# showlab/VideoSwap

Measured on AMD Instinct MI355X. Metric: denoised frames/sec, 16-frame 512x512 clip @ 50 DDIM steps (end to end: inversion + CFG sampling), higher is better.
Workload: dtype f16; 1 GPU; BASELINE.json configs[1]: 16-frame 512x512 clip, SD-1.5 UNet3D + AnimateDiff motion modules, 50-step DDIM inversion (B=1) + 50-step CFG-7.5 DDIM sampling (B=2), 1 clip per GPU per step; launch=eager, parallelism=clip-parallel x1

## Files before the change

videoswap_amd/csrc/gemm.hip:

```cpp
#include "gemm_common.h"
#include "prof.h"
#include <algorithm>
#include <cstdlib>
#include <stdlib.h>
#include <string.h>

using namespace vsxg;

static long tile_tune() { return vsxg::gemm_option("tile_tune"); }
static long force_tile() { return tile_tune() & 15; }
static bool tune_deep() { return (tile_tune() & 16) != 0; }
static int tune_splits() { return (int)((tile_tune() >> 8) & 15); }

namespace {


#ifdef VSX_GEMM_TIMING
#define TSTAMP(i) do { const long t_now = (long)clock64(); t_seg[i] += t_now - t_last; t_last = t_now; } while (0)
#else
#define TSTAMP(i) do { } while (0)
#endif

template <int BM, int BN, int WAVES_M, int WAVES_N, bool SWAP, int NSTAGE>
__global__ __launch_bounds__(WAVES_M* WAVES_N * 64) void gemm_kernel(const GemmParams p) {
    constexpr int PREFETCH = NSTAGE - 1;
    constexpr int NW = WAVES_M * WAVES_N;
    constexpr int WM = BM / WAVES_M, WN = BN / WAVES_N;
    constexpr int TM = WM / 32, TN = WN / 32;
    constexpr int A_BLKS = BM / 8, B_BLKS = BN / 8;
    static_assert(A_BLKS % NW == 0, "A blocks must split evenly over the waves");
    constexpr int GA = A_BLKS / NW;
    constexpr int GB_LO = B_BLKS / NW, GB_HI = (B_BLKS + NW - 1) / NW;
    constexpr int N_HI = B_BLKS - GB_LO * NW;
    constexpr int STAGE = (BM + BN) * 128;

    extern __shared__ __attribute__((aligned(16))) unsigned char smem[];

    const int tid = threadIdx.x;
    const int lane = tid & 63;
    const int wave = __builtin_amdgcn_readfirstlane(tid >> 6);
    const int wr = wave / WAVES_N, wc = wave % WAVES_N;
    const int l31 = lane & 31, hi = lane >> 5;
#ifdef VSX_GEMM_TIMING
    const long t_begin = (long)clock64();
#endif

    int tile_n, tile_m, split;
    if (p.xcd_gm > 0) {
        const int xcd = blockIdx.x & 7, local = blockIdx.x >> 3;
        const int gm = p.xcd_gm;
        const int RB = p.tiles_m / gm;
        const int CB = (p.tiles_n * (p.splitk > 1 ? p.splitk : 1)) / (8 / gm);
        const int lr = local % RB;
        const int np = (xcd / gm) * CB + local / RB;
        tile_m = (xcd % gm) * RB + lr;
        tile_n = np % p.tiles_n;
        split = np / p.tiles_n;
    } else {
        int wg = blockIdx.x;
        const int nwg = gridDim.x, q = nwg >> 3, r = nwg & 7;
        const int xcd = wg & 7, local = wg >> 3;
        wg = (xcd < r ? xcd * (q + 1) : r * (q + 1) + (xcd - r) * q) + local;
        tile_n = wg % p.tiles_n;
        tile_m = wg / p.tiles_n;
        split = p.splitk > 1 ? (int)blockIdx.z : 0;
    }
    const long m0 = (long)tile_m * BM;
    const long n0 = p.geglu ? (long)tile_n * (BN / 2) : (long)tile_n * BN;

    const int z = (p.splitk > 1 || p.xcd_gm > 0) ? 0 : (int)blockIdx.z;
    const int z0 = z / p.batch1, z1 = z - z0 * p.batch1;
    const half_t* Ab = p.A + z0 * p.a_bs0 + z1 * p.a_bs1;
    const half_t* Bb = p.B + z0 * p.b_bs0 + z1 * p.b_bs1;

    constexpr int OOB_OFF = (int)0x80000000;
    const int lrow = lane >> 3;
    const int pslot = lane & 7;
    const int kofs_e = (pslot ^ (lrow >> 1)) * 8;
    const int kofs_o = (pslot ^ (4 | (lrow >> 1))) * 8;

    const __amdgpu_buffer_rsrc_t rsrcA =
        __builtin_amdgcn_make_buffer_rsrc(const_cast<half_t*>(Ab), 0, (int)p.a_bytes, 0x00020000);
    const __amdgpu_buffer_rsrc_t rsrcA2 =
        __builtin_amdgcn_make_buffer_rsrc(const_cast<half_t*>(p.A2 ? p.A2 : p.A), 0, (int)p.a2_bytes, 0x00020000);
    const __amdgpu_buffer_rsrc_t rsrcB =
        __builtin_amdgcn_make_buffer_rsrc(const_cast<half_t*>(Bb), 0, (int)p.b_bytes, 0x00020000);

    bool a_ok[GA];
    int a_h0[GA], a_w0[GA], a_ibase[GA], a_kofs[GA];
    int va[GA];
    const int Hs = p.ups ? (p.H >> 1) : p.H;
    const int Ws = p.ups ? (p.W >> 1) : p.W;
    const int pad = p.pad;
#pragma unroll
    for (int i = 0; i < GA; ++i) {
        const long m = m0 + (wave * GA + i) * 8 + lrow;
        a_ok[i] = m < p.M;
        a_h0[i] = 0; a_w0[i] = 0; a_ibase[i] = 0;
        a_kofs[i] = ((wave * GA + i) & 1) ? kofs_o : kofs_e;
        va[i] = a_ok[i] ? (int)((m * p.lda + a_kofs[i]) * 2) : OOB_OFF;
        if (p.a_mode == 1) {
            const long hw = (long)p.Ho * p.Wo;
            const long mm = a_ok[i] ? m : 0;
            const int img = (int)(mm / hw);
            const int rem = (int)(mm - (long)img * hw);
            const int ho = rem / p.Wo;
            a_h0[i] = ho * p.stride - pad;
            a_w0[i] = (rem - ho * p.Wo) * p.stride - pad;
            a_ibase[i] = img * Hs;
        }
    }
    const int gbw = wave < N_HI ? GB_HI : GB_LO;
    const int b_blk0 = wave < N_HI ? wave * GB_HI : N_HI * GB_HI + (wave - N_HI) * GB_LO;
    int vb[GB_HI], b_kofs[GB_HI];
#pragma unroll
    for (int j = 0; j < GB_HI; ++j) {
        const int jr = (b_blk0 + j) * 8 + lrow;
        b_kofs[j] = ((b_blk0 + j) & 1) ? kofs_o : kofs_e;
        long n;
        bool ok;
        if (p.geglu) {
            const long oc = n0 + (jr >> 5) * 16 + (jr & 15);
            ok = oc < p.N;
            n = oc + ((jr & 16) ? p.N : 0);
        } else {
            n = n0 + jr;
            ok = n < p.N;
        }
        vb[j] = (ok && j < gbw) ? (int)((n * p.ldb + b_kofs[j]) * 2) : OOB_OFF;
    }

    const int Ctot = p.C1 + p.C2;
    const int nk = (int)((p.K + BK - 1) / BK);
    const int ktail_from = (int)(p.K - (long)(nk - 1) * BK);
    const bool fast_tap = p.a_mode == 1 && (Ctot % BK == 0) && (p.C1 % BK == 0);
    const int kt_begin = split * p.nk_per;
    const int kt_end = p.splitk > 1 ? min(nk, kt_begin + p.nk_per) : nk;
    int t_kh = 0, t_kw = 0, t_c = 0;
    bool t_second = false, t_dirty = true;
    if (fast_tap && kt_begin > 0) {
        const int k0 = kt_begin * BK;
        const int tap = k0 / Ctot, rem = k0 - tap * Ctot;
        t_kh = tap / p.ks;
        t_kw = tap - t_kh * p.ks;
        t_second = rem >= p.C1;
        t_c = t_second ? rem - p.C1 : rem;
    }

    unsigned char* i_sb = smem;
    bool i_tail = false, i_second = false;
    int i_soffA = 0, i_soffB = 0;
    auto issue_prep = [&](int kt, int stage) {
        unsigned char* sb = smem + stage * STAGE;
        const bool last_tail = (kt == nk - 1) && ktail_from < BK;
        int soffA = kt * (BK * 2), soffB = kt * (BK * 2);
        bool second = false;
        if (p.a_mode == 1) {
            if (fast_tap) {
                if (t_dirty) {
                    const int cs = t_second ? p.C2 : p.C1;
#pragma unroll
                    for (int i = 0; i < GA; ++i) {
                        const int hh = a_h0[i] + t_kh, ww = a_w0[i] + t_kw;
                        const bool ok = a_ok[i] && (unsigned)hh < (unsigned)p.H && (unsigned)ww < (unsigned)p.W;
                        const int hsrc = p.ups ? (hh >> 1) : hh, wsrc = p.ups ? (ww >> 1) : ww;
                        va[i] = ok ? (((a_ibase[i] + hsrc) * Ws + wsrc) * cs + a_kofs[i]) * 2 : OOB_OFF;
                    }
                    t_dirty = false;
                }
                second = t_second;
                soffA = t_c * 2;
                t_c += BK;
                if (t_c >= (t_second ? p.C2 : p.C1)) {
                    t_c = 0;
                    t_dirty = true;
                    if (!t_second && p.C2 > 0) {
                        t_second = true;
                    } else {
                        t_second = false;
                        if (++t_kw == p.ks) { t_kw = 0; ++t_kh; }
                    }
                }
            } else {
#pragma unroll
                for (int i = 0; i < GA; ++i) {
                    const long k = (long)kt * BK + a_kofs[i];
                    const int kk = k < p.K ? (int)k : 0;
                    const int tap = kk / Ctot;
                    const int ci = kk - tap * Ctot;
                    const int kh = tap / p.ks, kw = tap - kh * p.ks;
                    const int hh = a_h0[i] + kh, ww = a_w0[i] + kw;
                    const bool ok = a_ok[i] && k < p.K && (unsigned)hh < (unsigned)p.H && (unsigned)ww < (unsigned)p.W;
                    const int hsrc = p.ups ? (hh >> 1) : hh, wsrc = p.ups ? (ww >> 1) : ww;
                    va[i] = ok ? (((a_ibase[i] + hsrc) * Ws + wsrc) * p.C1 + ci) * 2 : OOB_OFF;
                }
                soffA = 0;
            }
        }
        i_sb = sb; i_tail = last_tail; i_second = second; i_soffA = soffA; i_soffB = soffB;
    };
    constexpr int NPIECE = GA + GB_HI;
    bool i_on = true;
    bool i_gate = true;
    auto issue_piece = [&](const int q) {
        if (!(i_on && i_gate)) return;
        if (q < GA) {
            const int qi = q < GA ? q : 0;
            const int v = (i_tail && a_kofs[qi] >= ktail_from) ? OOB_OFF : va[qi];
            lptr_t dst = (lptr_t)(i_sb + (wave * GA + q) * 1024);
            if (i_second)
                __builtin_amdgcn_raw_ptr_buffer_load_lds(rsrcA2, dst, 16, v, i_soffA, 0, 0);
            else
                __builtin_amdgcn_raw_ptr_buffer_load_lds(rsrcA, dst, 16, v, i_soffA, 0, 0);
        } else {
            const int j = q - GA;
            if (j < gbw) {
                const int jj = j < GB_HI ? j : 0;
                const int v = (i_tail && b_kofs[jj] >= ktail_from) ? OOB_OFF : vb[jj];
                __builtin_amdgcn_raw_ptr_buffer_load_lds(rsrcB, (lptr_t)(i_sb + BM * 128 + (b_blk0 + j) * 1024), 16, v,
                                                         i_soffB, 0, 0);
            }
        }
    };
    auto issue = [&](int kt, int stage) {
        issue_prep(kt, stage);
        i_on = true;
        i_gate = true;
#pragma unroll
        for (int q = 0; q < NPIECE; ++q) issue_piece(q);
    };

    constexpr int NACC = SWAP ? TN : TM, MACC = SWAP ? TM : TN;
    f16v acc[NACC][MACC];
#pragma unroll
    for (int i = 0; i < NACC; ++i)
#pragma unroll
        for (int j = 0; j < MACC; ++j)
#pragma unroll
            for (int r = 0; r < 16; ++r) acc[i][j][r] = 0.f;

    const int swz = (l31 >> 1) & 7;
    const int a_row = (wr * WM + l31) * 128;
    const int b_row = BM * 128 + (wc * WN + l31) * 128;
    int offs[4];
#pragma unroll
    for (int ks = 0; ks < 4; ++ks) offs[ks] = ((ks * 2 + hi) ^ swz) * 16;

    const int nloc = kt_end - kt_begin;
#pragma unroll
    for (int s = 0; s < PREFETCH; ++s)
        if (s < nloc) issue(kt_begin + s, s);

    constexpr bool PRE_RES = SWAP && (NW <= 8) && (TM * TN <= 5);
    constexpr int NRES = TM * TN * 2;
    h4 rpre[PRE_RES ? TM * TN * 4 : 1];
    const half_t* Rb0 = p.residual ? p.residual + z0 * p.r_bs0 + z1 * p.r_bs1 : nullptr;
    const bool pre_res = PRE_RES && Rb0 != nullptr && p.vec4 && !p.geglu && p.splitk <= 1;
    const bool res_late = pre_res && p.rvec8 && (int)n0 + BN <= (int)p.N;
    bool r_inflight = false;
    auto issue_residual = [&]() {
        if constexpr (PRE_RES) {
#pragma unroll
            for (int i = 0; i < TM; ++i) {
                const unsigned m = (unsigned)min((int)m0 + wr * WM + i * 32 + l31, (int)p.M - 1);
#pragma unroll
                for (int j = 0; j < TN; ++j)
#pragma unroll
                    for (int a = 0; a < 2; ++a) {
                        const int nc = (int)n0 + wc * WN + j * 32 + 16 * a + 8 * hi;
                        const uint4 v = *reinterpret_cast<const uint4*>(Rb0 + m * (unsigned)p.ldr + nc);
                        rpre[(i * TN + j) * 4 + 2 * a] = __builtin_bit_cast(h4, make_uint2(v.x, v.y));
                        rpre[(i * TN + j) * 4 + 2 * a + 1] = __builtin_bit_cast(h4, make_uint2(v.z, v.w));
                    }
            }
        }
    };
    const bool res_early = (p.pp_flags & TILE_RES_EARLY) != 0;
    const int kt_r = res_early ? 0 : max(nloc - 1 - PREFETCH, 0);
    bool r_loaded = false;
    auto wait_slab = [&](const int kt) {
        const int later = min(nloc - 1 - kt, PREFETCH - 1);
        if (PRE_RES && r_inflight) {
            if (wave < N_HI) {
                constexpr int G = GA + GB_HI;
                if (PREFETCH >= 3 && later >= 2) wait_vmcnt<2 * G + NRES>();
                else if (PREFETCH >= 2 && later == 1) wait_vmcnt<G + NRES>();
                else wait_vmcnt<NRES>();
            } else {
                constexpr int G = GA + GB_LO;
                if (PREFETCH >= 3 && later >= 2) wait_vmcnt<2 * G + NRES>();
                else if (PREFETCH >= 2 && later == 1) wait_vmcnt<G + NRES>();
                else wait_vmcnt<NRES>();
            }
            return;
        }
        if (wave < N_HI) {
            constexpr int G = GA + GB_HI;
            if (PREFETCH >= 3 && later >= 2) wait_vmcnt<2 * G>();
            else if (PREFETCH >= 2 && later == 1) wait_vmcnt<G>();
            else wait_vmcnt<0>();
        } else {
            constexpr int G = GA + GB_LO;
            if (PREFETCH >= 3 && later >= 2) wait_vmcnt<2 * G>();
            else if (PREFETCH >= 2 && later == 1) wait_vmcnt<G>();
            else wait_vmcnt<0>();
        }
    };
    auto ldfrag = [&](const unsigned char* sb, const int off, h8 (&af)[TM], h8 (&bf)[TN]) {
#pragma unroll
        for (int i = 0; i < TM; ++i) af[i] = *reinterpret_cast<const h8*>(sb + a_row + i * 4096 + off);
#pragma unroll
        for (int j = 0; j < TN; ++j) bf[j] = *reinterpret_cast<const h8*>(sb + b_row + j * 4096 + off);
    };
    auto mma = [&](const h8 (&af)[TM], const h8 (&bf)[TN]) {
#pragma unroll
        for (int i = 0; i < TM; ++i)
#pragma unroll
            for (int j = 0; j < TN; ++j) {
                if constexpr (SWAP)
                    acc[j][i] = __builtin_amdgcn_mfma_f32_32x32x16_f16(bf[j], af[i], acc[j][i], 0, 0, 0);
                else
                    acc[i][j] = __builtin_amdgcn_mfma_f32_32x32x16_f16(af[i], bf[j], acc[i][j], 0, 0, 0);
            }
    };

    auto mma_issue = [&](const h8 (&af)[TM], const h8 (&bf)[TN], const bool gate) {
        i_gate = gate;
#pragma unroll
        for (int i = 0; i < TM; ++i)
#pragma unroll
            for (int j = 0; j < TN; ++j) {
                if constexpr (SWAP)
                    acc[j][i] = __builtin_amdgcn_mfma_f32_32x32x16_f16(bf[j], af[i], acc[j][i], 0, 0, 0);
                else
                    acc[i][j] = __builtin_amdgcn_mfma_f32_32x32x16_f16(af[i], bf[j], acc[i][j], 0, 0, 0);
                if (i * TN + j < NPIECE) issue_piece(i * TN + j);
            }
#pragma unroll
        for (int q = TM * TN; q < NPIECE; ++q) issue_piece(q);
    };

#ifdef VSX_GEMM_TIMING
    long t_seg[4] = {0, 0, 0, 0}, t_last = 0, t_loop0 = 0;
#endif
    constexpr bool PIPE = (NW <= 8) && (TM * TN < 10);
    if constexpr (PIPE) {
        h8 af0[TM], bf0[TN], af1[TM], bf1[TN];
        wait_slab(0);
        __builtin_amdgcn_s_barrier();
        if (PREFETCH < nloc) issue(kt_begin + PREFETCH, PREFETCH & (NSTAGE - 1));
        ldfrag(smem, offs[0], af0, bf0);
        const bool late = NW >= 8 && wave >= NW / 2;
        i_on = false;
#ifdef VSX_GEMM_TIMING
        t_last = t_loop0 = (long)clock64();
#endif
        for (int kt = 0; kt + 1 < nloc; ++kt) {
            const unsigned char* sb = smem + (kt & (NSTAGE - 1)) * STAGE;
            ldfrag(sb, offs[1], af1, bf1);
            __builtin_amdgcn_sched_barrier(0);
            mma_issue(af0, bf0, late);
            __builtin_amdgcn_sched_barrier(0);
            if constexpr (PRE_RES) {
                if (res_late && kt == kt_r) {
                    issue_residual();
                    VSX_VMEM_NOTE(NRES);
                    r_inflight = !res_early;
                    r_loaded = true;
                }
                __builtin_amdgcn_sched_barrier(0);
            }
            ldfrag(sb, offs[2], af0, bf0);
            __builtin_amdgcn_sched_barrier(0);
            mma(af1, bf1);
            __builtin_amdgcn_sched_barrier(0);
            ldfrag(sb, offs[3], af1, bf1);
            __builtin_amdgcn_sched_barrier(0);
            mma(af0, bf0);
            __builtin_amdgcn_sched_barrier(0);
            TSTAMP(0);
            wait_slab(kt + 1);
            __builtin_amdgcn_s_waitcnt(0xC07F);
            TSTAMP(1);
            __builtin_amdgcn_s_barrier();
            TSTAMP(2);
            i_on = kt + 1 + PREFETCH < nloc;
            if (i_on) issue_prep(kt_begin + kt + 1 + PREFETCH, (kt + 1 + PREFETCH) & (NSTAGE - 1));
            ldfrag(smem + ((kt + 1) & (NSTAGE - 1)) * STAGE, offs[0], af0, bf0);
            __builtin_amdgcn_sched_barrier(0);
            mma_issue(af1, bf1, !late);
            __builtin_amdgcn_sched_barrier(0);
            TSTAMP(3);
        }
        if (nloc > 0) {
            const unsigned char* sb = smem + ((nloc - 1) & (NSTAGE - 1)) * STAGE;
            ldfrag(sb, offs[1], af1, bf1);
            mma(af0, bf0);
            ldfrag(sb, offs[2], af0, bf0);
            mma(af1, bf1);
            ldfrag(sb, offs[3], af1, bf1);
            mma(af0, bf0);
            mma(af1, bf1);
        }
    } else {
        const bool late16 = NW >= 16 && ((wave >> 2) & 1);
#ifdef VSX_GEMM_TIMING
        t_last = t_loop0 = (long)clock64();
#endif
        for (int kt = 0; kt < nloc; ++kt) {
            wait_slab(kt);
            TSTAMP(1);
            __builtin_amdgcn_s_barrier();
            TSTAMP(2);
            i_on = kt + PREFETCH < nloc;
            i_gate = true;
            if (i_on) issue_prep(kt_begin + kt + PREFETCH, (kt + PREFETCH) & (NSTAGE - 1));
            if (!late16) {
#pragma unroll
                for (int q = 0; q < NPIECE; ++q) issue_piece(q);
            }
            TSTAMP(3);
            const unsigned char* sb = smem + (kt & (NSTAGE - 1)) * STAGE;
#pragma unroll
            for (int ks = 0; ks < 4; ++ks) {
                h8 af[TM], bf[TN];
                ldfrag(sb, offs[ks], af, bf);
                mma(af, bf);
                if (ks == 0 && late16) {
#pragma unroll
                    for (int q = 0; q < NPIECE; ++q) issue_piece(q);
                }
            }
            TSTAMP(0);
        }
    }

#ifdef VSX_GEMM_TIMING
    long* const t_out = p.ws && p.splitk <= 1 ? reinterpret_cast<long*>(p.ws) + ((long)blockIdx.x * NW + wave) * 8 : nullptr;
    if (lane == 0 && t_out) {
        for (int k = 0; k < 4; ++k) t_out[k] = t_seg[k];
        t_out[4] = t_begin; t_out[5] = t_loop0; t_out[6] = (long)clock64();
    }
#define TSTAMP_END() do { asm volatile("s_waitcnt vmcnt(0)" ::: "memory"); if (lane == 0 && t_out) t_out[7] = (long)clock64(); } while (0)
#else
#define TSTAMP_END() do { } while (0)
#endif
    half_t* Cb = p.C + z0 * p.c_bs0 + z1 * p.c_bs1;
    const half_t* Rb = p.residual ? p.residual + z0 * p.r_bs0 + z1 * p.r_bs1 : nullptr;
    const int Mi = (int)p.M, Ni = (int)p.N;
    const int ldc = (int)p.ldc, ldr = (int)p.ldr;
    const int mb = (int)m0, nb0 = (int)n0;

    if constexpr (SWAP) {
        if (p.splitk > 1) {
            float* wsl = p.ws + (size_t)split * (size_t)Mi * (size_t)Ni;
#pragma unroll
            for (int i = 0; i < TM; ++i) {
                const int m = mb + wr * WM + i * 32 + l31;
                if (m >= Mi) continue;
#pragma unroll
                for (int j = 0; j < TN; ++j)
#pragma unroll
                    for (int g = 0; g < 4; ++g) {
                        const int nb = nb0 + wc * WN + j * 32 + 8 * g + 4 * hi;
                        if (nb + 3 < Ni) {
                            f4v o;
#pragma unroll
                            for (int e = 0; e < 4; ++e) o[e] = acc[j][i][4 * g + e] * p.alpha;
                            *reinterpret_cast<f4v*>(wsl + (size_t)m * Ni + nb) = o;
                        }
                    }
            }
            return;
        }
        constexpr bool PRE_BIAS = (NW <= 8) && (TM * TN <= 5);
        h4 bpre[PRE_BIAS ? TN : 1][4];
        const bool pre_bias = PRE_BIAS && p.bias != nullptr && p.vec8 && !p.geglu;
        if constexpr (PRE_BIAS) {
            if (pre_bias) {
#pragma unroll
                for (int j = 0; j < TN; ++j)
#pragma unroll
                    for (int g = 0; g < 4; ++g) {
                        const int nb = nb0 + wc * WN + j * 32 + 8 * g + 4 * hi;
                        bpre[j][g] = nb + 3 < Ni ? *reinterpret_cast<const h4*>(p.bias + nb) : h4{};
                    }
            }
        }
#pragma unroll
        for (int i = 0; i < TM; ++i) {
            const int m = mb + wr * WM + i * 32 + l31;
            if (m >= Mi) continue;
            const unsigned cbyte = (unsigned)m * (unsigned)ldc * 2u;
            const unsigned rbyte = (unsigned)m * (unsigned)ldr * 2u;
            const unsigned vbyte = p.rowvec ? ((unsigned)m / (unsigned)p.rows_per_vec) * (unsigned)Ni * 2u : 0u;
            const bool rrow = Rb != nullptr, rv = p.rowvec != nullptr;
            auto crow_at = [&](const int n) { return reinterpret_cast<half_t*>(reinterpret_cast<char*>(Cb) + (cbyte + 2u * (unsigned)n)); };
            auto rrow_at = [&](const int n) { return reinterpret_cast<const half_t*>(reinterpret_cast<const char*>(Rb) + (rbyte + 2u * (unsigned)n)); };
            auto rv_at = [&](const int n) { return reinterpret_cast<const half_t*>(reinterpret_cast<const char*>(p.rowvec) + (vbyte + 2u * (unsigned)n)); };
            const float* cvp = p.rowscale ? p.colvec : nullptr;
            const float rs = cvp ? p.rowscale[2 * (unsigned)m] : 1.f, rt = cvp ? p.rowscale[2 * (unsigned)m + 1] : 0.f;
            if (p.geglu) {
#pragma unroll
                for (int j = 0; j < TN; ++j) {
#pragma unroll
                    for (int q = 0; q < 2; ++q) {
                        const int nb = nb0 + (wc * TN + j) * 16 + 8 * q + 4 * hi;
                        if (nb >= Ni) continue;
                        float hv[4], gv[4];
// ... 221 lines not shown
}

__global__ __launch_bounds__(256) void splitk_reduce_kernel(const GemmParams p) {
    const long q = (long)blockIdx.x * 256 + threadIdx.x;
    const int nq = (int)(p.N >> 2);
    if (q >= p.M * nq) return;
    const int m = (int)(q / nq), nb = (int)(q - (long)m * nq) * 4;
    const size_t slab = (size_t)p.M * (size_t)p.N;
    f4v acc = *reinterpret_cast<const f4v*>(p.ws + (size_t)m * p.N + nb);
    for (int z = 1; z < p.splitk; ++z) {
        const f4v v = *reinterpret_cast<const f4v*>(p.ws + z * slab + (size_t)m * p.N + nb);
#pragma unroll
        for (int e = 0; e < 4; ++e) acc[e] += v[e];
    }
    if (p.rowscale) {
        const float rs = p.rowscale[2 * (size_t)m], rt = p.rowscale[2 * (size_t)m + 1];
        const f4v c = *reinterpret_cast<const f4v*>(p.colvec + nb);
#pragma unroll
        for (int e = 0; e < 4; ++e) acc[e] = __builtin_fmaf(rs, acc[e], rt * c[e]);
    }
    if (p.bias) {
        const h4 b = *reinterpret_cast<const h4*>(p.bias + nb);
#pragma unroll
        for (int e = 0; e < 4; ++e) acc[e] += (float)b[e];
    }
    if (p.rowvec) {
        const h4 b = *reinterpret_cast<const h4*>(p.rowvec + (size_t)(m / p.rows_per_vec) * p.N + nb);
#pragma unroll
        for (int e = 0; e < 4; ++e) acc[e] += (float)b[e];
    }
    if (p.residual) {
        const h4 b = *reinterpret_cast<const h4*>(p.residual + (size_t)m * p.ldr + nb);
#pragma unroll
        for (int e = 0; e < 4; ++e) acc[e] += (float)b[e];
    }
    h4 pk;
#pragma unroll
    for (int e = 0; e < 4; ++e) pk[e] = (half_t)acc[e];
    *reinterpret_cast<h4*>(p.C + (size_t)m * p.ldc + nb) = pk;
}

inline int plan_splitk(const vsx_gemm_desc* d, long tiles, bool eligible) {
    const long nk = (d->K + BK - 1) / BK;
    if (eligible && tune_splits() > 0) return tune_splits() <= nk ? tune_splits() : (int)nk;
    if (!eligible || tiles >= 160) return 1;
    int s = (int)((256 + tiles - 1) / tiles);
    if (s > 8) s = 8;
    while (s > 1 && nk / s < 12) --s;
    return s;
}

int plan_xcd_grid(const GemmParams& p, const long tiles_m, const int bm, const int bn, const long nbatch) {
    if (nbatch != 1 || gemm_option("xcd_walk") == 0) return 0;
    const int splits = p.splitk > 1 ? p.splitk : 1;
    const long np_total = (long)p.tiles_n * splits;
    if ((tiles_m * np_total) % 8 != 0 || tiles_m * np_total < 16) return 0;
    const long nk = (p.K + BK - 1) / BK;
    const double kslice = (double)(splits > 1 ? (long)p.nk_per * BK : nk * BK);
    const double taps = p.a_mode == 1 ? (double)(p.ks * p.ks) / (double)(p.stride * p.stride) : 1.0;
    const double a_panel = (double)bm * kslice * 2.0 / (taps < 1.0 ? 1.0 : taps);
    const double b_panel = (double)bn * kslice * 2.0;
    auto cost = [&](const int gm) -> double {
        const int gn = 8 / gm;
        if (tiles_m % gm != 0 || np_total % gn != 0) return -1.0;
        const long RB = tiles_m / gm, CB = np_total / gn;
        long nsp = 1;
        for (int b = 0; b < gn; ++b) {
            const long lo = b * CB, hi = lo + CB - 1;
            nsp = std::max(nsp, hi / p.tiles_n - lo / p.tiles_n + 1);
        }
        return (double)(RB * nsp) * a_panel + (double)CB * b_panel;
    };
    const double legacy = (tiles_m % 8 == 0) ? cost(8)
                                             : (double)((tiles_m + 7) / 8 + 1) * splits * a_panel + (double)np_total * b_panel;
    int best = 0;
    double best_cost = legacy;
    for (int gm = 4; gm >= 1; gm >>= 1) {
        const double c = cost(gm);
        if (c >= 0.0 && c < 0.95 * best_cost) { best = gm; best_cost = c; }
    }
    return best;
}

template <int BM, int BN, int WAVES_M, int WAVES_N, bool SWAP, int NSTAGE>
int launch(GemmParams& p, long tiles_m, long nbatch, hipStream_t stream) {
    constexpr size_t smem = (size_t)NSTAGE * (BM + BN) * 128;
    static_assert(smem <= 160 * 1024, "LDS ring exceeds 160 KiB");
    static bool attr_set = false;
    if (!attr_set) {
        hipError_t e = hipFuncSetAttribute(reinterpret_cast<const void*>(&gemm_kernel<BM, BN, WAVES_M, WAVES_N, SWAP, NSTAGE>),
                                           hipFuncAttributeMaxDynamicSharedMemorySize, (int)smem);
        if (e != hipSuccess) return vsx_fail(VSX_E_LAUNCH, "gemm: hipFuncSetAttribute: %s", hipGetErrorString(e));
        attr_set = true;
    }
    p.pp_flags = (int)(gemm_option("pp_sched") & TILE_RES_EARLY);
    p.tiles_m = (int)tiles_m;
    p.xcd_gm = plan_xcd_grid(p, tiles_m, BM, BN, nbatch);
    dim3 grid((unsigned)(tiles_m * p.tiles_n), 1, (unsigned)(p.splitk > 1 ? p.splitk : nbatch));
    if (p.xcd_gm > 0) grid = dim3((unsigned)(tiles_m * p.tiles_n * (p.splitk > 1 ? p.splitk : 1)), 1, 1);
    hipLaunchKernelGGL((gemm_kernel<BM, BN, WAVES_M, WAVES_N, SWAP, NSTAGE>), grid, dim3(WAVES_M * WAVES_N * 64), smem,
                       stream, p);
    return vsx_check_launch("vsx_gemm_f16");
}

template <int BM, int BN, int WAVES_M, int WAVES_N>
int launch_tile(GemmParams& p, long M, long cols, long nbatch, hipStream_t stream, bool deep = false) {
    p.tiles_n = (int)((cols + BN - 1) / BN);
    const long tiles_m = (M + BM - 1) / BM;
    constexpr int NST = ((BM + BN) * 128 * 4 <= 96 * 1024) ? 4 : 2;
    if constexpr (BM == 128 && BN == 160) {
        if (deep && p.c_mode != 1) return launch<BM, BN, WAVES_M, WAVES_N, true, 4>(p, tiles_m, nbatch, stream);
    }
    if (p.c_mode == 1) return launch<BM, BN, WAVES_M, WAVES_N, false, NST>(p, tiles_m, nbatch, stream);
    return launch<BM, BN, WAVES_M, WAVES_N, true, NST>(p, tiles_m, nbatch, stream);
}


int pp_mode() { return (int)gemm_option("gemm_pp"); }

enum GemmFamily { GEMM_WS, GEMM_PP256, GEMM_PP128, GEMM_TILE };
enum GemmRefusal { PLAN_OK = 0, PLAN_SUBPIXEL_OFF_PP, PLAN_ROWSTATS_PARTS };

struct GemmPlan {
    GemmFamily family;
    int BM, BN, WAVES_M, WAVES_N;
    bool deep;
    bool forced;
    long nbatch;
    int splits, nk_per;
    long stat_parts;
    int64_t workspace_bytes;
    GemmRefusal refused;
};

int fill_conv_params(const vsx_gemm_desc* d, GemmParams& p, const long nbatch) {
    VSX_REQUIRE(nbatch == 1, VSX_E_UNSUPPORTED, "gemm: conv mode does not take a batch");
    VSX_REQUIRE(d->ks == 1 || d->ks == 3, VSX_E_UNSUPPORTED, "gemm: conv kernel size %ld", (long)d->ks);
    VSX_REQUIRE(d->stride == 1 || d->stride == 2, VSX_E_UNSUPPORTED, "gemm: conv stride %ld", (long)d->stride);
    VSX_REQUIRE(d->C1 > 0 && d->C1 % 8 == 0 && d->C2 >= 0 && d->C2 % 8 == 0, VSX_E_BADSHAPE,
                "gemm: conv channels must be multiples of 8 (C1=%ld C2=%ld)", (long)d->C1, (long)d->C2);
    VSX_REQUIRE((d->C2 == 0) == (d->A2 == nullptr), VSX_E_BADSHAPE, "gemm: A2/C2 mismatch");
    VSX_REQUIRE(d->A2 == nullptr || vsx_aligned16(d->A2), VSX_E_BADSHAPE, "gemm: A2 must be 16-byte aligned");
    VSX_REQUIRE(d->K == d->ks * d->ks * (d->C1 + d->C2), VSX_E_BADSHAPE, "gemm: conv K mismatch");
    VSX_REQUIRE(d->C2 == 0 || (d->C1 % 64 == 0 && d->C2 % 64 == 0), VSX_E_UNSUPPORTED,
                "gemm: a two-source conv needs both channel counts to be multiples of 64 (one K slab)");
    VSX_REQUIRE(d->H > 0 && d->W > 0, VSX_E_BADSHAPE, "gemm: conv H/W");
    VSX_REQUIRE(!d->upsample || (d->H % 2 == 0 && d->W % 2 == 0), VSX_E_BADSHAPE, "gemm: upsample needs even H/W");
    p.H = (int)d->H; p.W = (int)d->W; p.C1 = (int)d->C1; p.C2 = (int)d->C2;
    p.ks = (int)d->ks; p.stride = (int)d->stride; p.ups = d->upsample ? 1 : 0;
    const bool subpix = d->upsample == 2;
    if (subpix) {
        VSX_REQUIRE(d->ks == 3 && d->stride == 1 && d->C2 == 0 && d->C1 % 64 == 0 && d->pad_lo < 0 && d->pad_hi < 0 &&
                        !d->rowvec && !d->residual && !d->geglu && d->c_mode == 0 && !d->rowscale && !d->rowstats,
                    VSX_E_UNSUPPORTED, "gemm: the sub-pixel form takes a single-source 3x3 stride-1 convolution with a bias only");
        VSX_REQUIRE(d->M % 4 == 0, VSX_E_BADSHAPE, "gemm: sub-pixel form: M must be a multiple of 4");
        p.ups = 0;
        p.H = (int)d->H / 2;
        p.W = (int)d->W / 2;
        p.sp_Mc = (int)(d->M / 4);
        p.K = 4 * d->C1;
    }
    const bool sym = d->pad_lo < 0 && d->pad_hi < 0;
    VSX_REQUIRE(sym || (d->pad_lo >= 0 && d->pad_hi >= 0 && d->pad_lo < d->ks && d->pad_hi < d->ks), VSX_E_BADSHAPE,
                "gemm: conv padding (%ld, %ld) for kernel size %ld", (long)d->pad_lo, (long)d->pad_hi, (long)d->ks);
    const int pad_lo = sym ? p.ks / 2 : (int)d->pad_lo, pad_hi = sym ? p.ks / 2 : (int)d->pad_hi;
    p.pad = pad_lo;
    p.Ho = (p.H + pad_lo + pad_hi - p.ks) / p.stride + 1;
    p.Wo = (p.W + pad_lo + pad_hi - p.ks) / p.stride + 1;
    {
        const long pix = (d->M / ((long)p.Ho * p.Wo) / (subpix ? 4 : 1)) * (long)(p.ups ? p.H / 2 : p.H) * (p.ups ? p.W / 2 : p.W);
        VSX_REQUIRE(pix * d->C1 * 2 < (1L << 31) && pix * d->C2 * 2 < (1L << 31), VSX_E_UNSUPPORTED,
                    "gemm: conv source tensors must be smaller than 2 GiB");
        p.a_bytes = (unsigned)(pix * d->C1 * 2);
        p.a2_bytes = (unsigned)(pix * d->C2 * 2);
    }
    VSX_REQUIRE(d->M % ((long)p.Ho * p.Wo) == 0, VSX_E_BADSHAPE, "gemm: conv M (%ld) not a multiple of Ho*Wo (%d*%d)",
                (long)d->M, p.Ho, p.Wo);
    if (subpix) {
        const long bb = ((4 * d->N - 1) * d->ldb + d->K) * 2;
        VSX_REQUIRE(bb < (1L << 31), VSX_E_UNSUPPORTED, "gemm: B operand slice must be smaller than 2 GiB");
        p.b_bytes = (unsigned)bb;
    }
    return VSX_OK;
}

void fill_vector_widths(const vsx_gemm_desc* d, GemmParams& p) {
    auto al8 = [](const void* q) { return (((uintptr_t)q) & 7) == 0; };
    p.vec4 = (d->ldc % 4 == 0 && d->c_bs0 % 4 == 0 && d->c_bs1 % 4 == 0 && al8(d->C) && al8(d->bias) &&
              al8(d->rowvec) && d->N % 4 == 0 &&
              (!d->residual || (al8(d->residual) && d->ldr % 4 == 0 && d->r_bs0 % 4 == 0 && d->r_bs1 % 4 == 0)))
                 ? 1 : 0;
    auto al16 = [](const void* q) { return (((uintptr_t)q) & 15) == 0; };
// ... 22 lines not shown
    p.B = (const half_t*)d->B;
    p.C = (half_t*)d->C;
    p.bias = (const half_t*)d->bias;
    p.rowvec = (const half_t*)d->rowvec;
    p.residual = (const half_t*)d->residual;
    p.rowscale = (const float*)d->rowscale;
    p.colvec = (const float*)d->colvec;
    VSX_REQUIRE((d->rowscale == nullptr) == (d->colvec == nullptr), VSX_E_BADSHAPE, "gemm: rowscale and colvec come together");
    VSX_REQUIRE(!d->rowscale || (d->batch0 * d->batch1 == 1 && d->a_mode == 0 && vsx_aligned16(d->colvec)), VSX_E_UNSUPPORTED,
                "gemm: rowscale / colvec (LayerNorm folded into a Linear) need an unbatched plain GEMM and a 16-byte aligned colvec");
    p.M = d->M; p.N = d->N; p.K = d->K;
    p.lda = d->lda; p.ldb = d->ldb; p.ldc = d->ldc; p.ldr = d->ldr;
    p.a_bs0 = d->a_bs0; p.a_bs1 = d->a_bs1; p.b_bs0 = d->b_bs0; p.b_bs1 = d->b_bs1;
    p.c_bs0 = d->c_bs0; p.c_bs1 = d->c_bs1; p.r_bs0 = d->r_bs0; p.r_bs1 = d->r_bs1;
    p.batch1 = (int)d->batch1;
    p.a_mode = (int)d->a_mode;
    p.geglu = (int)d->geglu;
    p.c_mode = (int)d->c_mode;
    p.alpha = (float)d->alpha;
    p.rows_per_vec = d->rows_per_vec > 0 ? d->rows_per_vec : 1;
    p.c_rows_per_img = d->c_rows_per_img;
    p.c_img_stride = d->c_img_stride;

    const long nbatch = d->batch0 * d->batch1;
    VSX_REQUIRE(d->M < (1L << 31) && d->N < (1L << 30) && (d->c_mode == 1 || d->M * d->ldc < (1L << 31)) &&
                    (!d->residual || d->M * d->ldr < (1L << 31)),
                VSX_E_UNSUPPORTED, "gemm: M*ldc and M*ldr must be below 2^31 elements");
    {
        const long brows = p.geglu ? 2 * d->N : d->N;
        const long bb = ((brows - 1) * d->ldb + d->K) * 2;
        VSX_REQUIRE(bb < (1L << 31), VSX_E_UNSUPPORTED, "gemm: B operand slice must be smaller than 2 GiB");
        p.b_bytes = (unsigned)bb;
    }
    VSX_REQUIRE(nbatch <= 65535, VSX_E_BADSHAPE, "gemm: batch0*batch1 = %ld exceeds 65535", nbatch);

    if (p.a_mode == 0) {
        VSX_REQUIRE(d->lda % 8 == 0, VSX_E_BADSHAPE, "gemm: lda (%ld) must be a multiple of 8", (long)d->lda);
        const long ab = ((d->M - 1) * d->lda + d->K) * 2;
        VSX_REQUIRE(ab < (1L << 31), VSX_E_UNSUPPORTED, "gemm: A operand slice must be smaller than 2 GiB");
        p.a_bytes = (unsigned)ab;
        p.a2_bytes = 0;
    } else if (p.a_mode == 1) {
        const int rc = fill_conv_params(d, p, nbatch);
        if (rc != VSX_OK) return rc;
    } else {
        return vsx_fail(VSX_E_UNSUPPORTED, "gemm: a_mode %d", p.a_mode);
    }
    if (p.c_mode == 1) {
        VSX_REQUIRE(!p.geglu && !d->rowvec && !d->residual, VSX_E_UNSUPPORTED, "gemm: transposed store takes bias only");
        VSX_REQUIRE(d->c_rows_per_img > 0, VSX_E_BADSHAPE, "gemm: c_rows_per_img");
        p.c_pack4 = (d->c_rows_per_img % 4 == 0 && d->ldc % 4 == 0 && d->c_img_stride % 4 == 0 &&
                     d->c_bs0 % 4 == 0 && d->c_bs1 % 4 == 0) ? 1 : 0;
    }
    if (p.geglu) VSX_REQUIRE(!d->rowvec, VSX_E_UNSUPPORTED, "gemm: geglu with rowvec");
    fill_vector_widths(d, p);
    return VSX_OK;
}

void set_tile(GemmPlan& plan, int bm, int bn, int waves_m, int waves_n, bool deep = false) {
    plan.family = GEMM_TILE;
    plan.BM = bm; plan.BN = bn; plan.WAVES_M = waves_m; plan.WAVES_N = waves_n;
    plan.deep = deep;
}

void plan_tile(const vsx_gemm_desc& d, const GemmParams& p, const int splits, const bool assume_workspace, GemmPlan& plan) {
    const long nbatch = d.batch0 * d.batch1;
    const long cols = p.geglu ? 2 * d.N : d.N;
    auto blocks = [&](long bm, long bn) { return ((d.M + bm - 1) / bm) * ((cols + bn - 1) / bn) * nbatch; };
    const bool wide = (cols % 320 == 0);
    const int64_t split_bytes = (int64_t)splits * d.M * d.N * (int64_t)sizeof(float);
    plan.forced = force_tile() && (wide || force_tile() >= 4);
    if (!plan.forced && splits > 1) plan.workspace_bytes = split_bytes;
    if (plan.forced) {
        if (force_tile() == 1) set_tile(plan, 128, 320, 4, 2);
        else if (force_tile() == 2) set_tile(plan, 128, 160, 4, 1, tune_deep());
        else if (force_tile() == 3) set_tile(plan, 256, 320, 8, 2);
        else if (force_tile() == 4) set_tile(plan, 128, 128, 2, 2);
        else if (force_tile() == 5) set_tile(plan, 64, 128, 2, 2);
        else set_tile(plan, 64, 64, 2, 2);
    } else if (splits > 1 && (assume_workspace || (d.workspace != nullptr && d.workspace_bytes >= split_bytes))) {
        const long nk = (d.K + BK - 1) / BK;
        plan.splits = splits;
        plan.nk_per = (int)((nk + splits - 1) / splits);
        set_tile(plan, 128, 320, 4, 2);
    } else if (wide && blocks(256, 320) >= 240 && (p.a_mode == 1 || p.geglu || p.residual == nullptr)) {
        set_tile(plan, 256, 320, 8, 2);
    } else if (cols % 160 == 0 && blocks(128, 160) >= 200) {
        set_tile(plan, 128, 160, 4, 1, blocks(128, 160) <= 256);
    } else if (cols % 160 == 0 && blocks(128, 160) >= 176 && !p.geglu && p.c_mode == 0) {
        set_tile(plan, 128, 160, 4, 1, true);
    } else if (wide && blocks(128, 320) >= 200) {
        set_tile(plan, 128, 320, 4, 2);
    } else if (blocks(128, 128) >= 512) {
        set_tile(plan, 128, 128, 2, 2);
    } else if (blocks(64, 128) >= 512 || (p.geglu && cols >= 128)) {
        set_tile(plan, 64, 128, 2, 2);
    } else {
        set_tile(plan, 64, 64, 2, 2);
    }
    if (p.c_mode == 1) plan.deep = false;
}

GemmPlan plan_gemm(const vsx_gemm_desc& d, const GemmParams& p, const bool assume_workspace) {
    GemmPlan plan{};
    plan.splits = 1;
    const long nbatch = plan.nbatch = d.batch0 * d.batch1;
    const long cols = p.geglu ? 2 * d.N : d.N;
    auto blocks = [&](long bm, long bn) { return ((d.M + bm - 1) / bm) * ((cols + bn - 1) / bn) * nbatch; };
    const bool wide = (cols % 320 == 0);
    const int splits = plan_splitk(&d, blocks(128, 320), wide && nbatch == 1 && !p.geglu && p.c_mode == 0 && p.vec4);
    const int pp = pp_mode();
    const bool pp_ok = pp != 0 && wide && nbatch == 1 && (splits <= 1 || pp >= 2) && !force_tile() && pp_supported(p);
    const long t128 = blocks(128, 320);
    const bool pp256 = pp_ok && pp != 3 && (blocks(256, 320) >= 192 || (pp == 2 && blocks(256, 320) >= 64) || pp == 4);
    const bool pp128 = !pp256 && pp_ok && p.c_mode != 1 && ((pp >= 2 && t128 >= 32) || (pp == 1 && p.a_mode != 1 && t128 >= 240 && t128 <= 272));
    const long ws_opt = gemm_option("gemm_ws");
    const bool ws_res = d.N == 320 && d.residual != nullptr && d.M >= (ws_opt == 3 ? 131072 : 65536);
    const bool ws_ln = ws_opt == 4 && d.N > 320 && d.rowscale != nullptr && d.M >= 65536;
    const bool ws_st = ws_opt == 5 && d.N == 320 && d.rowstats_parts >= 0 && d.rowscale == nullptr && d.residual == nullptr && d.M >= 131072;
    const bool ws = ws_opt != 0 && pp != 0 && nbatch == 1 && splits <= 1 && !force_tile() && ws_supported(p) && (ws_opt == 2 || ws_res || ws_ln || ws_st);
    plan.stat_parts = ws ? (p.rowscale ? 0 : (cols / 320) * ws_waves()) : ((pp256 || pp128) && pp_rowstats_ok(p) ? (cols / 320) * 6 : 0);
    if (d.rowstats != nullptr && !(plan.stat_parts > 0 && d.rowstats_parts == plan.stat_parts)) plan.refused = PLAN_ROWSTATS_PARTS;
    if (p.sp_Mc > 0 && !((pp256 && p.sp_Mc % 256 == 0) || (pp128 && p.sp_Mc % 128 == 0)) && !plan.refused)
        plan.refused = PLAN_SUBPIXEL_OFF_PP;
    if (ws) plan.family = GEMM_WS;
    else if (pp256) plan.family = GEMM_PP256;
    else if (pp128) plan.family = GEMM_PP128;
    else plan_tile(d, p, splits, assume_workspace, plan);
    return plan;
}

void gemm_work(const vsx_gemm_desc& d, const GemmParams& p, double* flop, double* bytes) {
    const long nbatch = d.batch0 * d.batch1;
    const long cols = p.geglu ? 2 * d.N : d.N;
    *flop = 2.0 * (double)d.M * (double)cols * (double)p.K * (double)nbatch;
    double a_el = (double)d.M * (double)d.K;
    if (p.a_mode == 1) {
        const double nimg = (double)d.M / ((double)p.Ho * (double)p.Wo) / (p.sp_Mc > 0 ? 4.0 : 1.0);
        const double hin = p.ups ? p.H / 2 : p.H, win = p.ups ? p.W / 2 : p.W;
        a_el = nimg * hin * win * (double)(p.C1 + p.C2);
    }
    const double w_el = (double)cols * (double)d.K * (p.sp_Mc > 0 ? 4.0 : 1.0);
    const double c_el = (double)d.M * (double)d.N;
    *bytes = 2.0 * (double)nbatch * (a_el + w_el + c_el + (d.residual ? c_el : 0.0));
}

template <int BM, int BN, int WAVES_M, int WAVES_N>
bool is_tile(const GemmPlan& plan) { return plan.BM == BM && plan.BN == BN && plan.WAVES_M == WAVES_M && plan.WAVES_N == WAVES_N; }

int run_plan(const GemmPlan& plan, GemmParams& p, hipStream_t stream) {
    if (plan.family == GEMM_WS) return launch_ws(p, stream);
    if (plan.family == GEMM_PP256) return launch_pp(p, 256, stream);
    if (plan.family == GEMM_PP128) return launch_pp(p, 128, stream);
    const long nbatch = plan.nbatch;
    const long cols = p.geglu ? 2 * p.N : p.N;
    if (plan.splits > 1) {
        p.splitk = plan.splits;
        p.nk_per = plan.nk_per;
    }
    int rc;
    if (is_tile<256, 320, 8, 2>(plan)) rc = launch_tile<256, 320, 8, 2>(p, p.M, cols, nbatch, stream);
    else if (is_tile<128, 320, 4, 2>(plan)) rc = launch_tile<128, 320, 4, 2>(p, p.M, cols, nbatch, stream);
    else if (is_tile<128, 160, 4, 1>(plan)) rc = launch_tile<128, 160, 4, 1>(p, p.M, cols, nbatch, stream, plan.deep);
    else if (is_tile<128, 128, 2, 2>(plan)) rc = launch_tile<128, 128, 2, 2>(p, p.M, cols, nbatch, stream);
    else if (is_tile<64, 128, 2, 2>(plan)) rc = launch_tile<64, 128, 2, 2>(p, p.M, cols, nbatch, stream);
    else if (is_tile<64, 64, 2, 2>(plan)) rc = launch_tile<64, 64, 2, 2>(p, p.M, cols, nbatch, stream);
// ... 51 lines not shown
```

videoswap_amd/csrc/gemm_common.h:

```cpp
#pragma once
#include "common.h"
#include "options.h"

namespace vsxg {

constexpr int BK = 64;

struct GemmParams {
    const half_t* A;
    const half_t* A2;
    const half_t* B;
    half_t* C;
    const half_t* bias;
    const half_t* rowvec;
    const half_t* residual;
    const float* rowscale;
    const float* colvec;
    float* rowstats;
    int rowstats_parts;
    long M, N, K;
    long lda, ldb, ldc, ldr;
    long a_bs0, a_bs1, b_bs0, b_bs1, c_bs0, c_bs1, r_bs0, r_bs1;
    long c_rows_per_img, c_img_stride, rows_per_vec;
    int batch1;
    int a_mode, H, W, C1, C2, Ho, Wo, ks, stride, ups, pad;
    int geglu, c_mode, c_pack4, vec4, vec8, rvec8;
    int tiles_n;
    unsigned a_bytes, a2_bytes, b_bytes;
    int splitk, nk_per;
    float* ws;
    float alpha;
    int tiles_total;
    int pp_flags;
    int sp_Mc;
    int xcd_gm, tiles_m;
};

constexpr int PP_TILES_LINEAR = 8;
constexpr int PP_CONV_TAP_MAJOR = 4;
constexpr int PP_CONV_PRIVATE_A = 16;
constexpr int PP_CONV_ASHIFT_ON = 1 << 16;
constexpr int PP_COMMON_ORDER = 32;
constexpr int TILE_RES_EARLY = 64;

typedef __attribute__((address_space(3))) void* lptr_t;

#ifndef VSX_VMEM_NOTE
#define VSX_VMEM_NOTE(n) do { } while (0)
#endif

#ifdef __HIPCC__
template <int N>
__device__ __forceinline__ void wait_vmcnt() {
    asm volatile("s_waitcnt vmcnt(%0)" ::"n"(N) : "memory");
}

#endif

bool pp_supported(const GemmParams& p);
bool pp_rowstats_ok(const GemmParams& p);
int launch_pp(GemmParams& p, int bm, hipStream_t stream);
bool ws_supported(const GemmParams& p);
int launch_ws(GemmParams& p, hipStream_t stream);
int ws_waves();

}
```

Baseline: 4.171 frames/s.

## Share one A slab across the three horizontal taps of 3x3 implicit-GEMM convs

Adds a SHARED variant of the implicit-GEMM conv kernel for 3x3 stride-1 pad-1 convs with power-of-two width. It loads the A (activation) slab once per kh/channel chunk and reuses it for all three kw taps. The kw offset is applied by shifting the LDS read row, and a small zeroed LDS region covers left/right edge pixels. This cuts global-to-LDS traffic for A by about three times, at the cost of reordering the K loop as channel-chunk × kh × kw. It also adds custom vmcnt wait logic and constraints on split-K chunking.

```diff
diff --git a/videoswap_amd/csrc/gemm.hip b/videoswap_amd/csrc/gemm.hip
--- a/videoswap_amd/csrc/gemm.hip
+++ b/videoswap_amd/csrc/gemm.hip
@@ -1,6 +1,7 @@
 #include "gemm_common.h"
 #include "prof.h"
 #include <algorithm>
+#include <type_traits>
 #include <cstdlib>
 #include <stdlib.h>
 #include <string.h>
@@ -21,9 +22,10 @@
 #define TSTAMP(i) do { } while (0)
 #endif
 
-template <int BM, int BN, int WAVES_M, int WAVES_N, bool SWAP, int NSTAGE>
+template <int BM, int BN, int WAVES_M, int WAVES_N, bool SWAP, int NSTAGE, bool SHARED = false>
 __global__ __launch_bounds__(WAVES_M* WAVES_N * 64) void gemm_kernel(const GemmParams p) {
     constexpr int PREFETCH = NSTAGE - 1;
+    constexpr int ZERO_OFF = NSTAGE * (BM + BN) * 128;
     constexpr int NW = WAVES_M * WAVES_N;
     constexpr int WM = BM / WAVES_M, WN = BN / WAVES_N;
     constexpr int TM = WM / 32, TN = WN / 32;
@@ -138,7 +140,13 @@
     const int kt_end = p.splitk > 1 ? min(nk, kt_begin + p.nk_per) : nk;
     int t_kh = 0, t_kw = 0, t_c = 0;
     bool t_second = false, t_dirty = true;
-    if (fast_tap && kt_begin > 0) {
+    if (SHARED && kt_begin > 0) {
+        const int n1 = 9 * (p.C1 / BK);
+        t_second = kt_begin >= n1;
+        const int j = t_second ? kt_begin - n1 : kt_begin;
+        t_c = (j / 9) * BK;
+        t_kh = (j % 9) / 3;
+    } else if (fast_tap && kt_begin > 0) {
         const int k0 = kt_begin * BK;
         const int tap = k0 / Ctot, rem = k0 - tap * Ctot;
         t_kh = tap / p.ks;
@@ -149,13 +157,36 @@
 
     unsigned char* i_sb = smem;
     bool i_tail = false, i_second = false;
+    bool i_hasA = true;
     int i_soffA = 0, i_soffB = 0;
     auto issue_prep = [&](int kt, int stage) {
         unsigned char* sb = smem + stage * STAGE;
         const bool last_tail = (kt == nk - 1) && ktail_from < BK;
         int soffA = kt * (BK * 2), soffB = kt * (BK * 2);
         bool second = false;
-        if (p.a_mode == 1) {
+        if constexpr (SHARED) {
+            i_hasA = t_kw == 0;
+            const int cs = t_second ? p.C2 : p.C1;
+            if (i_hasA) {
+#pragma unroll
+                for (int i = 0; i < GA; ++i) {
+                    const int hh = a_h0[i] + t_kh;
+                    const bool ok = a_ok[i] && (unsigned)hh < (unsigned)p.H;
+                    va[i] = ok ? (((a_ibase[i] + hh) * p.W + a_w0[i] + 1) * cs + a_kofs[i]) * 2 : OOB_OFF;
+                }
+            }
+            second = t_second;
+            soffA = t_c * 2;
+            soffB = ((t_kh * 3 + t_kw) * Ctot + (t_second ? p.C1 : 0) + t_c) * 2;
+            if (++t_kw == 3) {
+                t_kw = 0;
+                if (++t_kh == 3) {
+                    t_kh = 0;
+                    t_c += BK;
+                    if (t_c >= cs) { t_c = 0; t_second = true; }
+                }
+            }
+        } else if (p.a_mode == 1) {
             if (fast_tap) {
                 if (t_dirty) {
                     const int cs = t_second ? p.C2 : p.C1;
@@ -205,6 +236,7 @@
     auto issue_piece = [&](const int q) {
         if (!(i_on && i_gate)) return;
         if (q < GA) {
+            if (SHARED && !i_hasA) return;
             const int qi = q < GA ? q : 0;
             const int v = (i_tail && a_kofs[qi] >= ktail_from) ? OOB_OFF : va[qi];
             lptr_t dst = (lptr_t)(i_sb + (wave * GA + q) * 1024);
@@ -278,8 +310,31 @@
     const bool res_early = (p.pp_flags & TILE_RES_EARLY) != 0;
     const int kt_r = res_early ? 0 : max(nloc - 1 - PREFETCH, 0);
     bool r_loaded = false;
+    auto wait_shared = [&](const int kt, const int later, auto gb_c, auto nr_c) {
+        constexpr int GBW = decltype(gb_c)::value, NR = decltype(nr_c)::value;
+        const int ph = (int)((unsigned)kt % 3u);
+        if (PREFETCH >= 3 && later >= 2) {
+            if (ph != 0) wait_vmcnt<2 * GBW + GA + NR>(); else wait_vmcnt<2 * GBW + NR>();
+        } else if (PREFETCH >= 2 && later == 1) {
+            wait_vmcnt<GBW + NR>();
+        } else {
+            wait_vmcnt<NR>();
+        }
+    };
     auto wait_slab = [&](const int kt) {
         const int later = min(nloc - 1 - kt, PREFETCH - 1);
+        if constexpr (SHARED) {
+            using std::integral_constant;
+            const bool res = PRE_RES && r_inflight;
+            if (wave < N_HI) {
+                if (res) wait_shared(kt, later, integral_constant<int, GB_HI>{}, integral_constant<int, NRES>{});
+                else wait_shared(kt, later, integral_constant<int, GB_HI>{}, integral_constant<int, 0>{});
+            } else {
+                if (res) wait_shared(kt, later, integral_constant<int, GB_LO>{}, integral_constant<int, NRES>{});
+                else wait_shared(kt, later, integral_constant<int, GB_LO>{}, integral_constant<int, 0>{});
+            }
+            return;
+        }
         if (PRE_RES && r_inflight) {
             if (wave < N_HI) {
                 constexpr int G = GA + GB_HI;
@@ -306,9 +361,26 @@
             else wait_vmcnt<0>();
         }
     };
-    auto ldfrag = [&](const unsigned char* sb, const int off, h8 (&af)[TM], h8 (&bf)[TN]) {
-#pragma unroll
-        for (int i = 0; i < TM; ++i) af[i] = *reinterpret_cast<const h8*>(sb + a_row + i * 4096 + off);
+    int aoff[SHARED ? TM : 1];
+    const int wmask = SHARED ? p.W - 1 : 0;
+    auto shared_a_setup = [&](const int kt) {
+        const int kw = (int)((unsigned)kt % 3u);
+        const int r = l31 + kw - 1;
+        const int base = ((kt - kw) & (NSTAGE - 1)) * STAGE + (wr * WM + r) * 128 + ((hi ^ ((r >> 1) & 7)) * 16);
+#pragma unroll
+        for (int i = 0; i < (SHARED ? TM : 1); ++i) {
+            const int col = (wr * WM + i * 32 + l31) & wmask;
+            const bool edge = (kw == 0 && col == 0) || (kw == 2 && col == wmask);
+            aoff[i] = edge ? ZERO_OFF : base + i * 4096;
+        }
+    };
+    auto ldfrag = [&](const unsigned char* sb, const int ks, h8 (&af)[TM], h8 (&bf)[TN]) {
+        const int off = offs[ks];
+#pragma unroll
+        for (int i = 0; i < TM; ++i) {
+            if constexpr (SHARED) af[i] = *reinterpret_cast<const h8*>(smem + (aoff[i] ^ (ks * 32)));
+            else af[i] = *reinterpret_cast<const h8*>(sb + a_row + i * 4096 + off);
+        }
 #pragma unroll
         for (int j = 0; j < TN; ++j) bf[j] = *reinterpret_cast<const h8*>(sb + b_row + j * 4096 + off);
     };
@@ -344,12 +416,18 @@
     long t_seg[4] = {0, 0, 0, 0}, t_last = 0, t_loop0 = 0;
 #endif
     constexpr bool PIPE = (NW <= 8) && (TM * TN < 10);
+    static_assert(!SHARED || (PIPE && SWAP), "the shared A slab is built into the register-double-buffered loop only");
     if constexpr (PIPE) {
         h8 af0[TM], bf0[TN], af1[TM], bf1[TN];
+        if constexpr (SHARED) {
+            if (tid < 32) reinterpret_cast<float*>(smem + ZERO_OFF)[tid] = 0.f;
+            __builtin_amdgcn_s_waitcnt(0xC07F);
+            shared_a_setup(0);
+        }
         wait_slab(0);
         __builtin_amdgcn_s_barrier();
         if (PREFETCH < nloc) issue(kt_begin + PREFETCH, PREFETCH & (NSTAGE - 1));
-        ldfrag(smem, offs[0], af0, bf0);
+        ldfrag(smem, 0, af0, bf0);
         const bool late = NW >= 8 && wave >= NW / 2;
         i_on = false;
 #ifdef VSX_GEMM_TIMING
@@ -357,7 +435,7 @@
 #endif
         for (int kt = 0; kt + 1 < nloc; ++kt) {
             const unsigned char* sb = smem + (kt & (NSTAGE - 1)) * STAGE;
-            ldfrag(sb, offs[1], af1, bf1);
+            ldfrag(sb, 1, af1, bf1);
             __builtin_amdgcn_sched_barrier(0);
             mma_issue(af0, bf0, late);
             __builtin_amdgcn_sched_barrier(0);
@@ -370,11 +448,11 @@
                 }
                 __builtin_amdgcn_sched_barrier(0);
             }
-            ldfrag(sb, offs[2], af0, bf0);
+            ldfrag(sb, 2, af0, bf0);
             __builtin_amdgcn_sched_barrier(0);
             mma(af1, bf1);
             __builtin_amdgcn_sched_barrier(0);
-            ldfrag(sb, offs[3], af1, bf1);
+            ldfrag(sb, 3, af1, bf1);
             __builtin_amdgcn_sched_barrier(0);
             mma(af0, bf0);
             __builtin_amdgcn_sched_barrier(0);
@@ -386,7 +464,8 @@
             TSTAMP(2);
             i_on = kt + 1 + PREFETCH < nloc;
             if (i_on) issue_prep(kt_begin + kt + 1 + PREFETCH, (kt + 1 + PREFETCH) & (NSTAGE - 1));
-            ldfrag(smem + ((kt + 1) & (NSTAGE - 1)) * STAGE, offs[0], af0, bf0);
+            if constexpr (SHARED) shared_a_setup(kt + 1);
+            ldfrag(smem + ((kt + 1) & (NSTAGE - 1)) * STAGE, 0, af0, bf0);
             __builtin_amdgcn_sched_barrier(0);
             mma_issue(af1, bf1, !late);
             __builtin_amdgcn_sched_barrier(0);
@@ -394,11 +473,11 @@
         }
         if (nloc > 0) {
             const unsigned char* sb = smem + ((nloc - 1) & (NSTAGE - 1)) * STAGE;
-            ldfrag(sb, offs[1], af1, bf1);
+            ldfrag(sb, 1, af1, bf1);
             mma(af0, bf0);
-            ldfrag(sb, offs[2], af0, bf0);
+            ldfrag(sb, 2, af0, bf0);
             mma(af1, bf1);
-            ldfrag(sb, offs[3], af1, bf1);
+            ldfrag(sb, 3, af1, bf1);
             mma(af0, bf0);
             mma(af1, bf1);
         }
@@ -424,7 +503,7 @@
 #pragma unroll
             for (int ks = 0; ks < 4; ++ks) {
                 h8 af[TM], bf[TN];
-                ldfrag(sb, offs[ks], af, bf);
+                ldfrag(sb, ks, af, bf);
                 mma(af, bf);
                 if (ks == 0 && late16) {
 #pragma unroll
@@ -812,13 +891,21 @@
     return best;
 }
 
-template <int BM, int BN, int WAVES_M, int WAVES_N, bool SWAP, int NSTAGE>
+bool conv_shared_ok(const GemmParams& p, const int bm) {
+    if (p.a_mode != 1 || p.ks != 3 || p.stride != 1 || p.ups || p.sp_Mc > 0 || p.c_mode != 0) return false;
+    if (p.pad != 1 || p.Ho != p.H || p.Wo != p.W) return false;
+    if ((p.C1 + p.C2) % BK != 0 || p.C1 % BK != 0) return false;
+    if (p.W < 8 || (p.W & (p.W - 1)) != 0 || p.W > bm || bm > 128) return false;
+    return (gemm_option("pp_sched") & PP_CONV_TAP_MAJOR) == 0;
+}
+
+template <int BM, int BN, int WAVES_M, int WAVES_N, bool SWAP, int NSTAGE, bool SHARED = false>
 int launch(GemmParams& p, long tiles_m, long nbatch, hipStream_t stream) {
-    constexpr size_t smem = (size_t)NSTAGE * (BM + BN) * 128;
+    constexpr size_t smem = (size_t)NSTAGE * (BM + BN) * 128 + (SHARED ? 128 : 0);
     static_assert(smem <= 160 * 1024, "LDS ring exceeds 160 KiB");
     static bool attr_set = false;
     if (!attr_set) {
-        hipError_t e = hipFuncSetAttribute(reinterpret_cast<const void*>(&gemm_kernel<BM, BN, WAVES_M, WAVES_N, SWAP, NSTAGE>),
+        hipError_t e = hipFuncSetAttribute(reinterpret_cast<const void*>(&gemm_kernel<BM, BN, WAVES_M, WAVES_N, SWAP, NSTAGE, SHARED>),
                                            hipFuncAttributeMaxDynamicSharedMemorySize, (int)smem);
         if (e != hipSuccess) return vsx_fail(VSX_E_LAUNCH, "gemm: hipFuncSetAttribute: %s", hipGetErrorString(e));
         attr_set = true;
@@ -828,7 +915,7 @@
     p.xcd_gm = plan_xcd_grid(p, tiles_m, BM, BN, nbatch);
     dim3 grid((unsigned)(tiles_m * p.tiles_n), 1, (unsigned)(p.splitk > 1 ? p.splitk : nbatch));
     if (p.xcd_gm > 0) grid = dim3((unsigned)(tiles_m * p.tiles_n * (p.splitk > 1 ? p.splitk : 1)), 1, 1);
-    hipLaunchKernelGGL((gemm_kernel<BM, BN, WAVES_M, WAVES_N, SWAP, NSTAGE>), grid, dim3(WAVES_M * WAVES_N * 64), smem,
+    hipLaunchKernelGGL((gemm_kernel<BM, BN, WAVES_M, WAVES_N, SWAP, NSTAGE, SHARED>), grid, dim3(WAVES_M * WAVES_N * 64), smem,
                        stream, p);
     return vsx_check_launch("vsx_gemm_f16");
 }
@@ -838,6 +925,15 @@
     p.tiles_n = (int)((cols + BN - 1) / BN);
     const long tiles_m = (M + BM - 1) / BM;
     constexpr int NST = ((BM + BN) * 128 * 4 <= 96 * 1024) ? 4 : 2;
+    if constexpr (BM <= 128) {
+        p.conv_shared = conv_shared_ok(p, BM) && (p.splitk <= 1 || p.nk_per % 3 == 0) ? 1 : 0;
+        if (p.conv_shared) {
+            if constexpr (BM == 128 && BN == 160) {
+                if (deep) return launch<BM, BN, WAVES_M, WAVES_N, true, 4, true>(p, tiles_m, nbatch, stream);
+            }
+            return launch<BM, BN, WAVES_M, WAVES_N, true, NST, true>(p, tiles_m, nbatch, stream);
+        }
+    }
     if constexpr (BM == 128 && BN == 160) {
         if (deep && p.c_mode != 1) return launch<BM, BN, WAVES_M, WAVES_N, true, 4>(p, tiles_m, nbatch, stream);
     }
@@ -1026,6 +1122,7 @@
         const long nk = (d.K + BK - 1) / BK;
         plan.splits = splits;
         plan.nk_per = (int)((nk + splits - 1) / splits);
+        if (tune_splits() > 0 && conv_shared_ok(p, 128)) plan.nk_per = (plan.nk_per + 2) / 3 * 3;
         set_tile(plan, 128, 320, 4, 2);
     } else if (wide && blocks(256, 320) >= 240 && (p.a_mode == 1 || p.geglu || p.residual == nullptr)) {
         set_tile(plan, 256, 320, 8, 2);
diff --git a/videoswap_amd/csrc/gemm_common.h b/videoswap_amd/csrc/gemm_common.h
--- a/videoswap_amd/csrc/gemm_common.h
+++ b/videoswap_amd/csrc/gemm_common.h
@@ -34,6 +34,7 @@
     int pp_flags;
     int sp_Mc;
     int xcd_gm, tiles_m;
+    int conv_shared;
 };
 
 constexpr int PP_TILES_LINEAR = 8;
```

Result: no change. 4.204 frames/s, median of 6 (+0.8%).
